# chenxuhao/GraphAIBench

Hardware: AMD Instinct MI355X
Metric: GCN-layer fwd+bwd aggregated edges/sec (higher is better)
Workload: dtype f32; 1 GPU; ogbn-products-shaped Chung-Lu graph (seed 42), GCN hidden layer 128->128 fwd+bwd (2 SpMM D=128 + 3 dense products + relu/d_relu; 2 of the products ride on the SpMMs); nv=2449029, ne_with_selfloops=125915443, D=128, parallelism=1 GPU

## Files before the change

graphaibench_amd/csrc/spmm_core.h:

```cpp
#pragma once
#include <type_traits>
#include "common.h"

namespace {

struct SpmmArgs {
  const int64_t* rowptr;
  const uint32_t* col;
  const float* rw;
  const float* ew;
  const uint32_t* rev;
  const float* in;
  float* out;
  int64_t ld;
  int64_t ldo;
  int ncols;
  int n_rows;
  int heavy_thr;
  const uint32_t* row_list;
  const uint32_t* row_order;
  int nblocks;
  int per_xcd;
  int xcd_chunk;
  uint32_t in_bytes;
  const uint32_t* col_flagged;
  int accumulate;
  int relu;
  int heads;
  int dh;
  int compact;
  int col0;
  const uint32_t* row_map;
  const float* in2;
  uint32_t n_first;
  uint32_t in2_bytes;
};

template <bool PART>
__device__ __forceinline__ int64_t out_row(const SpmmArgs& a, int64_t r) {
  if constexpr (PART) return a.row_map ? (int64_t)a.row_map[r] : r;
  else return r;
}

template <int VEC> struct VecT;
template <> struct VecT<1> { typedef float type; };
template <> struct VecT<2> { typedef float type __attribute__((ext_vector_type(2))); };
template <> struct VecT<4> { typedef float type __attribute__((ext_vector_type(4))); };
template <> struct VecT<8> { typedef float type __attribute__((ext_vector_type(8))); };

template <int VEC>
__device__ __forceinline__ typename VecT<VEC>::type vzero() {
  typename VecT<VEC>::type z;
  if constexpr (VEC == 1) z = 0.f;
  else
    for (int i = 0; i < VEC; ++i) z[i] = 0.f;
  return z;
}
template <int VEC>
__device__ __forceinline__ typename VecT<VEC>::type vrelu(typename VecT<VEC>::type v) {
  if constexpr (VEC == 1) return v > 0.f ? v : 0.f;
  else {
#pragma unroll
    for (int i = 0; i < VEC; ++i) v[i] = v[i] > 0.f ? v[i] : 0.f;
    return v;
  }
}
template <int VEC>
__device__ __forceinline__ void vacc(typename VecT<VEC>::type& acc, float w,
                                     const typename VecT<VEC>::type& x) {
  if constexpr (VEC == 1) {
    float t = w * x;
    acc = acc + t;
  } else {
#pragma unroll
    for (int i = 0; i < VEC; ++i) {
      float t = w * x[i];
      acc[i] = acc[i] + t;
    }
  }
}

__device__ __forceinline__ int logical_block(const SpmmArgs& a) {
  int b = blockIdx.x;
  if (a.per_xcd > 0) {
    const int x = b & 7, k = b >> 3;
    if (a.xcd_chunk > 0) b = ((k / a.xcd_chunk) * 8 + x) * a.xcd_chunk + (k % a.xcd_chunk);
    else b = x * a.per_xcd + k;
  }
  return b;
}

template <int WMODE>
__device__ __forceinline__ float load_edge_w(const SpmmArgs& a, int64_t e, int head = 0) {
  if constexpr (WMODE == 1) return a.ew[e];
  else if constexpr (WMODE == 2) return a.ew[a.rev[e]];
  else if constexpr (WMODE == 3) return a.ew[e * a.heads + head];
  else if constexpr (WMODE == 4) return a.ew[(int64_t)a.rev[e] * a.heads + head];
  else return 0.f;
}

typedef unsigned u2_t __attribute__((ext_vector_type(2)));
typedef unsigned u4_t __attribute__((ext_vector_type(4)));

__device__ __forceinline__ float bf16_lo(unsigned w) { return __uint_as_float(w << 16); }
__device__ __forceinline__ float bf16_hi(unsigned w) { return __uint_as_float(w & 0xffff0000u); }
template <int VEC> struct Bf16Raw;
template <> struct Bf16Raw<1> { typedef unsigned short type; };
template <> struct Bf16Raw<2> { typedef unsigned type; };
template <> struct Bf16Raw<4> { typedef u2_t type; };
template <> struct Bf16Raw<8> { typedef u4_t type; };
template <int VEC>
__device__ __forceinline__ typename VecT<VEC>::type widen_bf16(typename Bf16Raw<VEC>::type r) {
  typename VecT<VEC>::type v;
  if constexpr (VEC == 1) v = __uint_as_float((unsigned)r << 16);
  else if constexpr (VEC == 2) {
    v[0] = bf16_lo(r);
    v[1] = bf16_hi(r);
  } else {
#pragma unroll
    for (int i = 0; i < VEC / 2; ++i) {
      v[2 * i] = bf16_lo(r[i]);
      v[2 * i + 1] = bf16_hi(r[i]);
    }
  }
  return v;
}
template <int VEC, typename E>
__device__ __forceinline__ typename VecT<VEC>::type load_elems(const char* p) {
  if constexpr (sizeof(E) == 4) return *reinterpret_cast<const typename VecT<VEC>::type*>(p);
  else return widen_bf16<VEC>(*reinterpret_cast<const typename Bf16Raw<VEC>::type*>(p));
}

struct zs_t { uint32_t bits; };
constexpr int GAIB_ZS_ROW_BYTES = 384;
constexpr int GAIB_ZS_CAP = 46;
struct zs_wide_t { uint32_t bits; };
template <typename E> struct ZsTraits { static constexpr bool zs = false; static constexpr uint32_t dense_row_bytes = 0u; };
template <> struct ZsTraits<zs_t> { static constexpr bool zs = true; static constexpr uint32_t dense_row_bytes = 512u; };
template <> struct ZsTraits<zs_wide_t> { static constexpr bool zs = true; static constexpr uint32_t dense_row_bytes = 1024u; };

template <int VEC, int GM, bool PART = false, typename E = float>
struct RowGather {
  static constexpr bool BUF = GM != 0;
  static constexpr bool ZS = ZsTraits<E>::zs;
  static_assert(!PART || !ZS, "two-table gathers: fp32 or bf16 tables");
  static_assert(!ZS || (VEC == 2 && (GM == 1 || GM == 3)), "zero-suppressed tables: 8-byte lanes (128 columns), buffer addressing");
  __amdgpu_buffer_rsrc_t rsrc, rsrc2;
  const char *inb, *inb2;
  int64_t ldb;
  uint32_t n_first;
  __device__ __forceinline__ RowGather(const SpmmArgs& a) {
    inb = reinterpret_cast<const char*>(a.in);
    ldb = a.ld * (int64_t)sizeof(E);
    if constexpr (BUF) rsrc = __builtin_amdgcn_make_buffer_rsrc((void*)a.in, 0, (int)a.in_bytes, 0x00020000);
    if constexpr (PART) {
      n_first = a.in2 ? a.n_first : 0xffffffffu;
      inb2 = reinterpret_cast<const char*>(a.in2) - (int64_t)a.n_first * ldb;
      if constexpr (BUF) rsrc2 = __builtin_amdgcn_make_buffer_rsrc((void*)a.in2, 0, (int)a.in2_bytes, 0x00020000);
    }
    if constexpr (ZS) rsrc2 = __builtin_amdgcn_make_buffer_rsrc((void*)a.in2, 0, (int)a.in2_bytes, 0x00020000);
  }
  typedef typename std::conditional<ZS, u2_t, typename std::conditional<sizeof(E) == 2, typename Bf16Raw<VEC>::type,
                                                                           typename VecT<VEC>::type>::type>::type raw_t;
  static __device__ __forceinline__ typename VecT<VEC>::type widen(const raw_t& r) {
    static_assert(!ZS, "zero-suppressed tables are expanded by zs_issue / zs_select");
    if constexpr (sizeof(E) == 2) return widen_bf16<VEC>(r);
    else return r;
  }
  typedef unsigned long long zs_mask_t;
  static __device__ __forceinline__ uint32_t zs_over_bits(zs_mask_t m0, zs_mask_t m1) {
    return ((uint32_t)__builtin_popcountll(m0) + (uint32_t)(63 - GAIB_ZS_CAP)) | ((uint32_t)__builtin_popcountll(m1) + (uint32_t)(63 - GAIB_ZS_CAP));
  }
  static __device__ __forceinline__ bool zs_over(uint32_t over) { return (over & 64u) != 0; }
  static __device__ __forceinline__ void zs_issue(const raw_t& r, raw_t& p, zs_mask_t& m0, zs_mask_t& m1, uint32_t& over) {
    m0 = ((zs_mask_t)(uint32_t)__builtin_amdgcn_readlane((int)r[1], 0) << 32) | (uint32_t)__builtin_amdgcn_readlane((int)r[0], 0);
    m1 = ((zs_mask_t)(uint32_t)__builtin_amdgcn_readlane((int)r[1], 1) << 32) | (uint32_t)__builtin_amdgcn_readlane((int)r[0], 1);
    over |= zs_over_bits(m0, m1);
    const uint32_t l0 = __builtin_amdgcn_mbcnt_hi((uint32_t)(m0 >> 32), __builtin_amdgcn_mbcnt_lo((uint32_t)m0, 2u));
    const uint32_t l1 = __builtin_amdgcn_mbcnt_hi((uint32_t)(m1 >> 32), __builtin_amdgcn_mbcnt_lo((uint32_t)m1, 2u));
    p[0] = (uint32_t)__builtin_amdgcn_ds_bpermute((int)(l0 << 2), (int)r[0]);
    p[1] = (uint32_t)__builtin_amdgcn_ds_bpermute((int)(l1 << 2), (int)r[1]);
  }
  __device__ __forceinline__ typename VecT<VEC>::type zs_fix(const raw_t& p, zs_mask_t m0, zs_mask_t m1, uint32_t cvec, int idx, uint32_t voff) const {
    if (zs_over(zs_over_bits(m0, m1))) {
      const uint32_t cf = (uint32_t)__builtin_amdgcn_readlane((int)cvec, idx);
      const uint32_t cj = GM == 3 ? (cf & 0x7fffffffu) : cf;
      u2_t d;
      if (GM == 3 && (cf & 0x80000000u))
        d = __builtin_amdgcn_raw_buffer_load_b64(rsrc2, (int)voff, (int)(cj * ZsTraits<E>::dense_row_bytes), 2);
      else d = __builtin_amdgcn_raw_buffer_load_b64(rsrc2, (int)voff, (int)(cj * ZsTraits<E>::dense_row_bytes), 0);
      typename VecT<VEC>::type v;
      v[0] = __uint_as_float(d[0]);
      v[1] = __uint_as_float(d[1]);
      return v;
    }
    return zs_select(p, m0, m1);
  }
  static __device__ __forceinline__ typename VecT<VEC>::type zs_select(const raw_t& r, zs_mask_t m0, zs_mask_t m1) {
    uint32_t k0, k1;
    asm("v_cndmask_b32_e64 %0, 0, %1, %2" : "=v"(k0) : "v"(r[0]), "s"(m0));
    asm("v_cndmask_b32_e64 %0, 0, %1, %2" : "=v"(k1) : "v"(r[1]), "s"(m1));
    typename VecT<VEC>::type v;
    v[0] = __uint_as_float(k0);
    v[1] = __uint_as_float(k1);
    return v;
  }
  __device__ __forceinline__ typename VecT<VEC>::type load(uint32_t cj, uint32_t voff) const { return widen(load_raw(cj, voff)); }
  __device__ __forceinline__ raw_t load_raw(uint32_t cj, uint32_t voff) const {
    typedef typename VecT<VEC>::type vec_t;
    if constexpr (PART) {
      static_assert(GM == 0 || GM == 1, "two-table gathers: plain buffer or global loads");
      const bool second = cj >= n_first;
      if constexpr (GM == 1) {
        const int soff = (int)((second ? cj - n_first : cj) * (uint32_t)ldb);
        return load_rsrc<0>(second ? rsrc2 : rsrc, soff, voff);
      } else {
        const char* rowp = (second ? inb2 : inb) + (int64_t)cj * ldb;
        return *reinterpret_cast<const raw_t*>(rowp + voff);
      }
    } else if constexpr (ZS) {
      const int zoff = (int)(voff < (uint32_t)GAIB_ZS_ROW_BYTES ? voff : 0u);
      if constexpr (GM == 3) {
        const uint32_t c = cj & 0x7fffffffu;
        if (cj & 0x80000000u) return __builtin_amdgcn_raw_buffer_load_b64(rsrc, zoff, (int)(c * (uint32_t)GAIB_ZS_ROW_BYTES), 2);
        return __builtin_amdgcn_raw_buffer_load_b64(rsrc, zoff, (int)(c * (uint32_t)GAIB_ZS_ROW_BYTES), 0);
      } else {
        return __builtin_amdgcn_raw_buffer_load_b64(rsrc, zoff, (int)(cj * (uint32_t)GAIB_ZS_ROW_BYTES), 0);
      }
    } else if constexpr (GM == 3) {
      const uint32_t c = cj & 0x7fffffffu;
      if (cj & 0x80000000u) return load_buf<2>(c, voff);
      return load_buf<0>(c, voff);
    } else if constexpr (GM == 2) {
      return load_buf<2>(cj, voff);
    } else if constexpr (GM == 1) {
      return load_buf<0>(cj, voff);
    } else {
      const char* rowp = inb + (int64_t)cj * ldb;
      if constexpr (sizeof(E) == 2) return *reinterpret_cast<const raw_t*>(rowp + voff);
      else return *reinterpret_cast<const vec_t*>(rowp + voff);
    }
  }
  template <int AUX>
  __device__ __forceinline__ raw_t load_buf(uint32_t cj, uint32_t voff) const {
    return load_rsrc<AUX>(rsrc, (int)(cj * (uint32_t)ldb), voff);
  }
  template <int AUX>
  __device__ __forceinline__ raw_t load_rsrc(__amdgpu_buffer_rsrc_t rsrc, int soff, uint32_t voff) const {
    typedef typename VecT<VEC>::type vec_t;
    if constexpr (sizeof(E) == 2) {
      if constexpr (VEC == 1) return __builtin_amdgcn_raw_buffer_load_b16(rsrc, (int)voff, soff, AUX);
      else if constexpr (VEC == 2) return __builtin_amdgcn_raw_buffer_load_b32(rsrc, (int)voff, soff, AUX);
      else if constexpr (VEC == 4) return __builtin_amdgcn_raw_buffer_load_b64(rsrc, (int)voff, soff, AUX);
      else return __builtin_amdgcn_raw_buffer_load_b128(rsrc, (int)voff, soff, AUX);
    } else if constexpr (VEC == 1) {
      return __uint_as_float(__builtin_amdgcn_raw_buffer_load_b32(rsrc, (int)voff, soff, AUX));
    } else if constexpr (VEC == 2) {
      u2_t r = __builtin_amdgcn_raw_buffer_load_b64(rsrc, (int)voff, soff, AUX);
      vec_t v;
      v[0] = __uint_as_float(r[0]);
      v[1] = __uint_as_float(r[1]);
      return v;
    } else {
      u4_t r = __builtin_amdgcn_raw_buffer_load_b128(rsrc, (int)voff, soff, AUX);
      vec_t v;
#pragma unroll
      for (int i = 0; i < 4; ++i) v[i] = __uint_as_float(r[i]);
      return v;
    }
  }
};

#ifndef GAIB_ZS_GROUP
#define GAIB_ZS_GROUP 4
#endif

template <int G, int CT, int WMODE, int U, typename gather_t>
__device__ __forceinline__ void zs_accumulate_group(const gather_t& gather, const typename gather_t::raw_t (&x)[U][CT], int xo, uint32_t c, float w,
                                                    float roww, int j0, const uint32_t (&voff)[CT], typename VecT<2>::type (&acc)[CT]) {
  typename gather_t::zs_mask_t m0[G][CT], m1[G][CT];
  typename gather_t::raw_t p[G][CT];
  uint32_t over = 0u;
#pragma unroll
  for (int u = 0; u < G; ++u)
#pragma unroll
    for (int ct = 0; ct < CT; ++ct) gather_t::zs_issue(x[xo + u][ct], p[u][ct], m0[u][ct], m1[u][ct], over);
  if (__builtin_expect(gather_t::zs_over(over), 0)) {
#pragma unroll
    for (int u = 0; u < G; ++u) {
      const float wj = (WMODE == 0) ? roww : readlane_f(w, j0 + u);
#pragma unroll
      for (int ct = 0; ct < CT; ++ct) {
        const typename VecT<2>::type t = gather.zs_fix(p[u][ct], m0[u][ct], m1[u][ct], c, j0 + u, voff[ct]) * wj;
        acc[ct] = acc[ct] + t;
      }
    }
  } else {
#pragma unroll
    for (int u = 0; u < G; ++u) {
      const float wj = (WMODE == 0) ? roww : readlane_f(w, j0 + u);
#pragma unroll
      for (int ct = 0; ct < CT; ++ct) {
        const typename VecT<2>::type t = gather_t::zs_select(p[u][ct], m0[u][ct], m1[u][ct]) * wj;
        acc[ct] = acc[ct] + t;
      }
    }
  }
}

template <int VEC, int CT, int WMODE, int U, int BUF, bool PART = false, bool PRE = false, typename E = float>
__device__ __forceinline__ void wave_accumulate(const SpmmArgs& a, int lane, int64_t eb, int64_t ee,
                                                int64_t chunk_stride, float roww,
                                                const uint32_t (&voff)[CT],
                                                typename VecT<VEC>::type (&acc)[CT], uint32_t c_first = 0u,
                                                float w_first = 0.f) {
  static_assert((sizeof(E) == 4 && !ZsTraits<E>::zs) || WMODE < 3, "bf16 and zero-suppressed tables: single-head weights");
  typedef RowGather<VEC, BUF, PART, E> gather_t;
  const gather_t gather(a);
  typename gather_t::raw_t x[U][CT];
  constexpr bool MH = WMODE >= 3;
  int hd[CT];
  float wv[MH ? U : 1][CT];
#pragma unroll
  for (int ct = 0; ct < CT; ++ct) {
    if constexpr (MH) hd[ct] = (int)(((uint32_t)a.col0 + (voff[ct] >> 2)) / (uint32_t)a.dh);
    else hd[ct] = 0;
  }
  for (int64_t base = eb; base < ee; base += chunk_stride) {
    const int64_t rem = ee - base;
    const int n = rem < 64 ? (int)rem : 64;
    uint32_t c = 0;
    float w = 0.f;
    if (PRE && base == eb) {
      c = c_first;
      w = w_first;
    } else if (lane < n) {
      c = a.col[base + lane];
      if constexpr (WMODE == 1 || WMODE == 2) w = load_edge_w<WMODE>(a, base + lane);
    }
    int j = 0;
    for (; j + U <= n; j += U) {
#pragma unroll
      for (int u = 0; u < U; ++u) {
        const uint32_t cj = (uint32_t)__builtin_amdgcn_readlane((int)c, j + u);
#pragma unroll
        for (int ct = 0; ct < CT; ++ct) {
          x[u][ct] = gather.load_raw(cj, voff[ct]);
          if constexpr (MH) wv[u][ct] = load_edge_w<WMODE>(a, base + j + u, hd[ct]);
        }
      }
      __builtin_amdgcn_sched_barrier(0);
      if constexpr (gather_t::ZS) {
        constexpr int H = GAIB_ZS_GROUP < U ? GAIB_ZS_GROUP : U;
#pragma unroll
        for (int u = 0; u < U; u += H) zs_accumulate_group<H, CT, WMODE>(gather, x, u, c, w, roww, j + u, voff, acc);
      } else {
#pragma unroll
        for (int u = 0; u < U; ++u) {
          const float wj = (WMODE == 0) ? roww : (MH ? 0.f : readlane_f(w, j + u));
#pragma unroll
          for (int ct = 0; ct < CT; ++ct) {
            float wsel = wj;
            if constexpr (MH) wsel = wv[u][ct];
            vacc<VEC>(acc[ct], wsel, gather_t::widen(x[u][ct]));
          }
        }
      }
    }
    const int r = n - j;
    if (r > 0) {
      int jj = j;
#pragma unroll
      for (int p = U / 2; p >= 1; p >>= 1) {
        if (r & p) {
#pragma unroll
          for (int u = 0; u < p; ++u) {
            const uint32_t cj = (uint32_t)__builtin_amdgcn_readlane((int)c, jj + u);
#pragma unroll
            for (int ct = 0; ct < CT; ++ct) x[p + u][ct] = gather.load_raw(cj, voff[ct]);
          }
          jj += p;
        }
      }
      __builtin_amdgcn_sched_barrier(0);
      jj = j;
#pragma unroll
      for (int p = U / 2; p >= 1; p >>= 1) {
        if (r & p) {
          if constexpr (gather_t::ZS) {
            if (p >= GAIB_ZS_GROUP) {
#pragma unroll
              for (int u = 0; u < p; u += GAIB_ZS_GROUP)
                zs_accumulate_group<GAIB_ZS_GROUP, CT, WMODE>(gather, x, p + u, c, w, roww, jj + u, voff, acc);
            } else if (p == 8) zs_accumulate_group<8, CT, WMODE>(gather, x, p, c, w, roww, jj, voff, acc);
            else if (p == 4) zs_accumulate_group<4, CT, WMODE>(gather, x, p, c, w, roww, jj, voff, acc);
            else if (p == 2) zs_accumulate_group<2, CT, WMODE>(gather, x, p, c, w, roww, jj, voff, acc);
            else zs_accumulate_group<1, CT, WMODE>(gather, x, p, c, w, roww, jj, voff, acc);
          } else {
#pragma unroll
            for (int u = 0; u < p; ++u) {
              const float wj = (WMODE == 0) ? roww : (MH ? 0.f : readlane_f(w, jj + u));
#pragma unroll
              for (int ct = 0; ct < CT; ++ct) {
                float wh = wj;
                if constexpr (MH) wh = load_edge_w<WMODE>(a, base + jj + u, hd[ct]);
                vacc<VEC>(acc[ct], wh, gather_t::widen(x[p + u][ct]));
              }
            }
          }
          jj += p;
        }
      }
    }
  }
}

}
```

graphaibench_amd/csrc/spmm_kernels.h:

```cpp
#pragma once
#include <algorithm>
#include "spmm_core.h"

namespace {

template <int VEC, int CT, int WMODE, int U, int BUF, bool PART = false, typename E = float>
__global__ __launch_bounds__(256) void spmm_w64_kernel(SpmmArgs a) {
  typedef typename VecT<VEC>::type vec_t;
  const int lane = threadIdx.x & 63;
  const int lb = logical_block(a);
  if (lb >= a.nblocks) return;
  int row = lb * 4 + (threadIdx.x >> 6);
  if (row >= a.n_rows) return;
  row = __builtin_amdgcn_readfirstlane(row);
  const int64_t e0 = a.rowptr[row], e1 = a.rowptr[row + 1];
  if (e1 - e0 > (int64_t)a.heavy_thr) return;
  bool colok[CT];
  uint32_t voff[CT];
  vec_t acc[CT];
#pragma unroll
  for (int ct = 0; ct < CT; ++ct) {
    colok[ct] = (lane + ct * 64) * VEC < a.ncols;
    voff[ct] = colok[ct] ? (uint32_t)((lane + ct * 64) * VEC * (int)sizeof(E)) : 0u;
    acc[ct] = vzero<VEC>();
  }
  const float roww = (WMODE == 0) ? a.rw[row] : 0.f;
  float* o = a.out + out_row<PART>(a, row) * a.ldo + lane * VEC;
  if (a.accumulate) {
#pragma unroll
    for (int ct = 0; ct < CT; ++ct)
      if (colok[ct]) acc[ct] = *reinterpret_cast<const vec_t*>(o + ct * 64 * VEC);
  }
  wave_accumulate<VEC, CT, WMODE, U, BUF, PART, false, E>(a, lane, e0, e1, 64, roww, voff, acc);
#pragma unroll
  for (int ct = 0; ct < CT; ++ct)
    if (colok[ct]) *reinterpret_cast<vec_t*>(o + ct * 64 * VEC) = a.relu ? vrelu<VEC>(acc[ct]) : acc[ct];
}

constexpr int HEAVY_WAVES = 16;
template <int VEC, int CT, int WMODE, int U, int BUF, bool PART = false, typename E = float>
__global__ __launch_bounds__(HEAVY_WAVES * 64) void spmm_heavy_kernel(SpmmArgs a) {
  typedef typename VecT<VEC>::type vec_t;
  extern __shared__ __attribute__((aligned(16))) float red[];
  const int lane = threadIdx.x & 63;
  const int wave = threadIdx.x >> 6;
  const int slot = (int)a.row_order[blockIdx.x];
  const int row = (int)a.row_list[slot];
  const int64_t e0 = a.rowptr[row], e1 = a.rowptr[row + 1];
  uint32_t voff[CT];
  vec_t acc[CT];
#pragma unroll
  for (int ct = 0; ct < CT; ++ct) {
    const bool ok = (lane + ct * 64) * VEC < a.ncols;
    voff[ct] = ok ? (uint32_t)((lane + ct * 64) * VEC * (int)sizeof(E)) : 0u;
    acc[ct] = vzero<VEC>();
  }
  const float roww = (WMODE == 0) ? a.rw[row] : 0.f;
  wave_accumulate<VEC, CT, WMODE, U, BUF, PART, false, E>(a, lane, e0 + (int64_t)wave * 64, e1,
                                                          (int64_t)HEAVY_WAVES * 64, roww, voff, acc);
  constexpr int W = CT * 64 * VEC;
#pragma unroll
  for (int ct = 0; ct < CT; ++ct)
    *reinterpret_cast<vec_t*>(&red[wave * W + (ct * 64 + lane) * VEC]) = acc[ct];
  __syncthreads();
  float* orow = a.out + (a.compact ? (int64_t)slot : out_row<PART>(a, row)) * a.ldo;
  for (int c = threadIdx.x; c < a.ncols; c += HEAVY_WAVES * 64) {
    float s = a.accumulate ? orow[c] + red[c] : red[c];
#pragma unroll
    for (int w = 1; w < HEAVY_WAVES; ++w) s = s + red[w * W + c];
    orow[c] = (a.relu && !(s > 0.f)) ? 0.f : s;
  }
}

template <int VEC, int G, int WMODE, typename E = float>
__global__ __launch_bounds__(256) void spmm_sub_kernel(SpmmArgs a) {
  typedef typename VecT<VEC>::type vec_t;
  constexpr int RPW = 64 / G;
  constexpr int U = 4;
  const int lane = threadIdx.x & 63;
  const int sub = lane / G, sl = lane % G;
  const int lb = logical_block(a);
  if (lb >= a.nblocks) return;
  const int64_t row = ((int64_t)lb * 4 + (threadIdx.x >> 6)) * RPW + sub;
  int64_t e0 = 0, e1 = 0;
  bool active = row < a.n_rows;
  if (active) {
    e0 = a.rowptr[row];
    e1 = a.rowptr[row + 1];
    if (e1 - e0 > (int64_t)a.heavy_thr) { active = false; e1 = e0; }
  }
  const bool colok = sl * VEC < a.ncols;
  vec_t acc = vzero<VEC>();
  if (a.accumulate && active && colok) acc = *reinterpret_cast<const vec_t*>(a.out + row * a.ldo + sl * VEC);
  const float roww = (WMODE == 0 && active) ? a.rw[row] : 0.f;
  const int head = (WMODE >= 3 && colok) ? (sl * VEC) / a.dh : 0;
  const float* inl = a.in + sl * VEC;
  const char* inl_e = reinterpret_cast<const char*>(a.in) + sl * VEC * (int)sizeof(E);
  for (int64_t e = e0; e < e1; e += U) {
    uint32_t cj[U];
    float wj[U];
    vec_t x[U];
#pragma unroll
    for (int u = 0; u < U; ++u) {
      const bool ok = e + u < e1;
      cj[u] = ok ? a.col[e + u] : 0u;
      wj[u] = (WMODE == 0) ? roww : (ok ? load_edge_w<WMODE>(a, e + u, head) : 0.f);
    }
#pragma unroll
    for (int u = 0; u < U; ++u) {
      const bool ok = e + u < e1;
      if constexpr (sizeof(E) == 2)
        x[u] = (ok && colok) ? load_elems<VEC, E>(inl_e + (int64_t)cj[u] * a.ld * 2) : vzero<VEC>();
      else
        x[u] = (ok && colok) ? *reinterpret_cast<const vec_t*>(inl + (int64_t)cj[u] * a.ld) : vzero<VEC>();
    }
#pragma unroll
    for (int u = 0; u < U; ++u)
      if (e + u < e1) vacc<VEC>(acc, wj[u], x[u]);
  }
  if (active && colok) *reinterpret_cast<vec_t*>(a.out + row * a.ldo + sl * VEC) = a.relu ? vrelu<VEC>(acc) : acc;
}

template <int VEC, int CT, int WMODE, int U, int BUF, bool PART = false, typename E = float>
int launch_w64_u(gaib_ctx* ctx, const gaib_graph* g, SpmmArgs a) {
  constexpr double EB = sizeof(E);
  if (g->n_heavy > 0) {
    SpmmArgs h = a;
    h.row_list = g->heavy_rows;
    h.row_order = g->heavy_rows + g->n_heavy;
    size_t lds = sizeof(float) * HEAVY_WAVES * CT * 64 * VEC;
    ProfScope ps(ctx, sizeof(E) == 2 ? "spmm_bf16_heavy" : "spmm_heavy",
                 gaib_alg_spmm_bytes((double)g->heavy_edges, (double)g->n_heavy, a.ncols, WMODE == 0 ? 0 : 4, a.accumulate ? 2 : 1, EB),
                 2.0 * g->heavy_edges * a.ncols, a.ncols);
    constexpr int UH = (WMODE >= 3 && U * CT * VEC > 16) ? (U / 2 > 4 ? U / 2 : 4) : U;
    spmm_heavy_kernel<VEC, CT, WMODE, UH, BUF, PART, E><<<dim3((unsigned)g->n_heavy), HEAVY_WAVES * 64, lds,
                                                         ctx->stream>>>(h);
    GAIB_LAUNCH_CHECK();
  }
  a.nblocks = (int)cdiv64(a.n_rows, 4);
  unsigned grid = (unsigned)a.nblocks;
  if (ctx->spmm_xcd_swizzle && a.nblocks >= 64) {
    a.per_xcd = (int)cdiv64(a.nblocks, 8);
    if (ctx->spmm_xcd_swizzle == 2 && a.nblocks >= 8 * 64) {
      a.xcd_chunk = 64;
      a.per_xcd = (int)(cdiv64(a.per_xcd, 64) * 64);
    }
    grid = (unsigned)a.per_xcd * 8u;
  }
  if (grid > 0) {
    const double e_l = (double)g->ne - (g->n_heavy > 0 ? (double)g->heavy_edges : 0.0), r_l = (double)a.n_rows - (double)g->n_heavy;
    ProfScope ps(ctx, sizeof(E) == 2 ? (!PART ? "spmm_bf16_light" : (a.in2 ? "part_bf16_light_2t" : (a.accumulate ? "part_bf16_light_acc" : "part_bf16_light")))
                                     : (!PART ? "spmm_light" : (a.in2 ? "part_light_2t" : (a.accumulate ? "part_light_acc" : "part_light"))),
                 gaib_alg_spmm_bytes(e_l, r_l, a.ncols, WMODE == 0 ? 0 : 4, a.accumulate ? 2 : 1, EB), 2.0 * e_l * a.ncols, a.ncols);
    spmm_w64_kernel<VEC, CT, WMODE, U, BUF, PART, E><<<dim3(grid), 256, 0, ctx->stream>>>(a);
    GAIB_LAUNCH_CHECK();
  }
  return GAIB_OK;
}

template <int VEC, int CT, int WMODE, typename E = float>
int launch_w64(gaib_ctx* ctx, const gaib_graph* g, SpmmArgs a) {
  constexpr int U = (VEC * CT >= 8) ? 4 : (VEC * CT >= 4 ? 8 : 16);
  int gm = (a.in_bytes != 0 && ctx->spmm_addr_mode != 2) ? 1 : 0;
  if (gm == 1 && ctx->spmm_gather_mode == 2) gm = 2;
  if (gm == 1 && ctx->spmm_gather_mode == 3 && a.col_flagged) {
    gm = 3;
    a.col = a.col_flagged;
  }
  if constexpr (U > 8) {
    if (ctx->spmm_unroll == 8) {
      switch (gm) {
        case 0: return launch_w64_u<VEC, CT, WMODE, 8, 0, false, E>(ctx, g, a);
        case 2: return launch_w64_u<VEC, CT, WMODE, 8, 2, false, E>(ctx, g, a);
        case 3: return launch_w64_u<VEC, CT, WMODE, 8, 3, false, E>(ctx, g, a);
        default: return launch_w64_u<VEC, CT, WMODE, 8, 1, false, E>(ctx, g, a);
      }
    }
  }
  switch (gm) {
    case 0: return launch_w64_u<VEC, CT, WMODE, U, 0, false, E>(ctx, g, a);
    case 2: return launch_w64_u<VEC, CT, WMODE, U, 2, false, E>(ctx, g, a);
    case 3: return launch_w64_u<VEC, CT, WMODE, U, 3, false, E>(ctx, g, a);
    default: return launch_w64_u<VEC, CT, WMODE, U, 1, false, E>(ctx, g, a);
  }
}

template <int VEC, int G, int WMODE, typename E = float>
int launch_sub(gaib_ctx* ctx, const gaib_graph* g, SpmmArgs a) {
  if (g->n_heavy > 0) {
    SpmmArgs h = a;
    h.row_list = g->heavy_rows;
    h.row_order = g->heavy_rows + g->n_heavy;
    size_t lds = sizeof(float) * HEAVY_WAVES * 64 * VEC;
    ProfScope ps(ctx, sizeof(E) == 2 ? "spmm_bf16_heavy" : "spmm_heavy",
                 gaib_alg_spmm_bytes((double)g->heavy_edges, (double)g->n_heavy, a.ncols, WMODE == 0 ? 0 : 4, a.accumulate ? 2 : 1,
                                     (double)sizeof(E)), 2.0 * g->heavy_edges * a.ncols, a.ncols);
    constexpr int UH = VEC >= 8 ? 4 : 8;
    spmm_heavy_kernel<VEC, 1, WMODE, UH, 0, false, E><<<dim3((unsigned)g->n_heavy), HEAVY_WAVES * 64, lds,
                                                         ctx->stream>>>(h);
    GAIB_LAUNCH_CHECK();
  }
  constexpr int RPW = 64 / G;
  a.nblocks = (int)cdiv64(a.n_rows, 4 * RPW);
  unsigned grid = (unsigned)a.nblocks;
  if (ctx->spmm_xcd_swizzle && a.nblocks >= 64) {
    a.per_xcd = (int)cdiv64(a.nblocks, 8);
    grid = (unsigned)a.per_xcd * 8u;
  }
  if (grid > 0) {
    const double e_l = (double)g->ne - (g->n_heavy > 0 ? (double)g->heavy_edges : 0.0), r_l = (double)a.n_rows - (double)g->n_heavy;
    ProfScope ps(ctx, sizeof(E) == 2 ? "spmm_bf16_sub" : "spmm_sub",
                 gaib_alg_spmm_bytes(e_l, r_l, a.ncols, WMODE == 0 ? 0 : 4, a.accumulate ? 2 : 1, (double)sizeof(E)), 2.0 * e_l * a.ncols,
                 a.ncols);
    spmm_sub_kernel<VEC, G, WMODE, E><<<dim3(grid), 256, 0, ctx->stream>>>(a);
    GAIB_LAUNCH_CHECK();
  }
  return GAIB_OK;
}

template <int VEC, int WMODE>
int dispatch_ct(gaib_ctx* ctx, const gaib_graph* g, const SpmmArgs& a, int lanes) {
  if (lanes <= 64) return launch_w64<VEC, 1, WMODE>(ctx, g, a);
  if (lanes <= 128) return launch_w64<VEC, 2, WMODE>(ctx, g, a);
  if constexpr (VEC == 4) {
    gaib_set_error("spmm: %d 16-byte lanes in one launch (internal: the slab width is 128 lanes at VEC = 4)", lanes);
    return GAIB_ERR_INVALID;
  } else {
    return launch_w64<VEC, 4, WMODE>(ctx, g, a);
  }
}

template <int VEC, int WMODE>
int dispatch_sub(gaib_ctx* ctx, const gaib_graph* g, const SpmmArgs& a, int lanes) {
  if (lanes <= 1) return launch_sub<VEC, 1, WMODE>(ctx, g, a);
  if (lanes <= 2) return launch_sub<VEC, 2, WMODE>(ctx, g, a);
  if (lanes <= 4) return launch_sub<VEC, 4, WMODE>(ctx, g, a);
  if (lanes <= 8) return launch_sub<VEC, 8, WMODE>(ctx, g, a);
  if (lanes <= 16) return launch_sub<VEC, 16, WMODE>(ctx, g, a);
  return launch_sub<VEC, 32, WMODE>(ctx, g, a);
}

template <int WMODE>
int dispatch_vec(gaib_ctx* ctx, const gaib_graph* g, const SpmmArgs& a0, int len) {
  const uintptr_t al = (uintptr_t)a0.in | (uintptr_t)a0.out;
  int vmax = 1;
  if (len % 4 == 0 && (al & 15) == 0) vmax = 4;
  else if (len % 2 == 0 && (al & 7) == 0) vmax = 2;
  if (WMODE >= 3) {
    while (vmax > 1 && a0.dh % vmax != 0) vmax >>= 1;
  }
  int variant = ctx->spmm_variant;
  const int lanes_max = (len + vmax - 1) / vmax;
  bool use_sub = false;
  int vec = vmax;
  if (len <= 64) vec = 1;
  else if (len <= 256 && vmax >= 2) vec = 2;
  else if (len <= 128) vec = 1;
  if (WMODE >= 3 && a0.dh % vec != 0) vec = 1;
  if (variant == 1) { use_sub = false; vec = 1; }
  if (variant == 2 && vmax >= 2) { use_sub = false; vec = 2; }
  if (variant == 4 && vmax >= 4) { use_sub = false; vec = 4; }
  if (variant == 32 && lanes_max <= 32) { use_sub = true; vec = vmax; }
  if (use_sub) {
    SpmmArgs a = a0;
    a.ncols = len;
    const int lanes = (len + vec - 1) / vec;
    if (vec == 4) return dispatch_sub<4, WMODE>(ctx, g, a, lanes);
    if (vec == 2) return dispatch_sub<2, WMODE>(ctx, g, a, lanes);
    return dispatch_sub<1, WMODE>(ctx, g, a, lanes);
  }
  const int slab = (vec == 4 ? 128 : 256) * vec;
  for (int c0 = 0; c0 < len; c0 += slab) {
    SpmmArgs a = a0;
    a.in = a0.in + c0;
    a.out = a0.out + c0;
    a.col0 = c0;
    if (a.in_bytes) a.in_bytes -= (uint32_t)(c0 * 4);
    a.ncols = (len - c0 < slab) ? (len - c0) : slab;
    const int lanes = (a.ncols + vec - 1) / vec;
    int rc;
    if (vec == 4) rc = dispatch_ct<4, WMODE>(ctx, g, a, lanes);
    else if (vec == 2) rc = dispatch_ct<2, WMODE>(ctx, g, a, lanes);
    else rc = dispatch_ct<1, WMODE>(ctx, g, a, lanes);
    if (rc != GAIB_OK) return rc;
  }
  return GAIB_OK;
}

struct FuseArgs {
  const float* wt;
  float* y;
  int64_t ldy;
  int n_out;
  int relu;
  const float* heavy_agg;
  const uint32_t* heavy_rows;
  int n_heavy;
  int* tile_counter;
  const float* agg_in;
  const float* wt2;
  const float* rows2;
  int ldw;
  int y_accum;
  int overlaps_transfer;
  int tile_xcd;
};

static int tile_xcd_arg(gaib_ctx* ctx, gaib_graph* g) {
  int v = ctx->spmm_tile_xcd;
  if (v < 0) {
    if (gaib_graph_ensure_locality(ctx, g) != GAIB_OK) return 0;
    v = g->near_frac >= 0.25f ? 1024 : 0;
  }
  if (v <= 0) return 0;
  if (v == 1) v = 16;
  int sh = 0;
  while ((2 << sh) <= v) ++sh;
  return sh + 1;
}

typedef float f32x4_t __attribute__((ext_vector_type(4)));
constexpr int FUSE_ROWS = 16;
constexpr int FUSE_WAVES = 16;

template <int VEC, int WMODE, int U, int GM, int STRIP, bool DUAL, bool FLAT = false, bool YACC = false, bool PART = false,
          bool RING = false, bool AFFINE = false, bool PREF = false, typename E = float>
__global__ __launch_bounds__(FUSE_WAVES * 64) void spmm_gemm_kernel(SpmmArgs a, FuseArgs f) {
  typedef typename VecT<VEC>::type vec_t;
  typedef RowGather<VEC, GM, PART, E> gather_t;
  constexpr int K = 64 * VEC;
  constexpr int KQ = K / 4;
  constexpr int LDT = K + 4;
  constexpr int HALF = STRIP;
  constexpr int NPASS = FUSE_ROWS / STRIP;
  extern __shared__ __attribute__((aligned(16))) float fuse_lds[];
  const int lane = threadIdx.x & 63;
  const int wave = threadIdx.x >> 6;
  const int n_pad = (f.n_out + 15) & ~15;
  float* wl = fuse_lds;
  float* wl2 = fuse_lds + n_pad * LDT;
  float* tile = fuse_lds + (DUAL ? 2 : 1) * n_pad * LDT + wave * (HALF * LDT);
  for (int t = threadIdx.x; t < n_pad * K; t += FUSE_WAVES * 64) {
    const int n = t / K, k = t % K;
    const bool in = n < f.n_out && k < a.ncols;
    wl[n * LDT + k] = in ? f.wt[(int64_t)n * f.ldw + k] : 0.f;
    if constexpr (DUAL) wl2[n * LDT + k] = in ? f.wt2[(int64_t)n * f.ldw + k] : 0.f;
  }
  __syncthreads();
  const int i = lane & 15, kq = lane >> 4;
  const bool colok = lane * VEC < a.ncols;
  auto store_row = [&](vec_t* p, const vec_t& v) { __builtin_nontemporal_store(v, p); };
  const uint32_t voff[1] = {colok ? (uint32_t)(lane * VEC * (int)sizeof(E)) : 0u};
  const int ntiles = (a.n_rows + FUSE_ROWS - 1) / FUSE_ROWS;
  const int tsh = AFFINE ? f.tile_xcd - 1 : 0;
  int own = AFFINE ? (int)(blockIdx.x & 7) : 0;
  int k_next = 0, k_left = 0;
  const int nwaves4 = ((int)gridDim.x * FUSE_WAVES * 4) / 8 > 0 ? ((int)gridDim.x * FUSE_WAVES * 4) / 8 : 1;
  const int per_xcd_tiles = (ntiles + 7) / 8;
  const int n_chunks = AFFINE ? (ntiles + (1 << tsh) - 1) >> tsh : 0;
  for (;;) {
    if (k_left == 0) {
      int want = 1;
// ... 553 lines not shown
```

Before: 14.69 billion edges/s.

## Software-pipeline zero-suppressed gathers by refilling buffers during group accumulation

In the zero-suppressed gather path with U=16, the edge loop now preloads the first 16 neighbor rows. After each 4-wide group's decode is issued, it starts loading the matching rows of the next chunk, so memory latency overlaps with accumulation. The remainder (tail) loads are also placed into freed slots during the last full chunk. The heavy-row kernel opts out and keeps the old loop. This costs more register pressure and a more complex tail-slot mapping, which could lower occupancy.

```diff
diff --git a/graphaibench_amd/csrc/spmm_core.h b/graphaibench_amd/csrc/spmm_core.h
--- a/graphaibench_amd/csrc/spmm_core.h
+++ b/graphaibench_amd/csrc/spmm_core.h
@@ -275,9 +275,13 @@
 #define GAIB_ZS_GROUP 4
 #endif
 
-template <int G, int CT, int WMODE, int U, typename gather_t>
+struct ZsNoRefill {
+  __device__ __forceinline__ void operator()() const {}
+};
+template <int G, int CT, int WMODE, int U, typename gather_t, typename refill_t = ZsNoRefill>
 __device__ __forceinline__ void zs_accumulate_group(const gather_t& gather, const typename gather_t::raw_t (&x)[U][CT], int xo, uint32_t c, float w,
-                                                    float roww, int j0, const uint32_t (&voff)[CT], typename VecT<2>::type (&acc)[CT]) {
+                                                    float roww, int j0, const uint32_t (&voff)[CT], typename VecT<2>::type (&acc)[CT],
+                                                    const refill_t& refill = refill_t()) {
   typename gather_t::zs_mask_t m0[G][CT], m1[G][CT];
   typename gather_t::raw_t p[G][CT];
   uint32_t over = 0u;
@@ -285,6 +289,10 @@
   for (int u = 0; u < G; ++u)
 #pragma unroll
     for (int ct = 0; ct < CT; ++ct) gather_t::zs_issue(x[xo + u][ct], p[u][ct], m0[u][ct], m1[u][ct], over);
+  if constexpr (!std::is_same<refill_t, ZsNoRefill>::value) {
+    refill();
+    __builtin_amdgcn_sched_barrier(0);
+  }
   if (__builtin_expect(gather_t::zs_over(over), 0)) {
 #pragma unroll
     for (int u = 0; u < G; ++u) {
@@ -308,7 +316,7 @@
   }
 }
 
-template <int VEC, int CT, int WMODE, int U, int BUF, bool PART = false, bool PRE = false, typename E = float>
+template <int VEC, int CT, int WMODE, int U, int BUF, bool PART = false, bool PRE = false, typename E = float, bool ROLL = true>
 __device__ __forceinline__ void wave_accumulate(const SpmmArgs& a, int lane, int64_t eb, int64_t ee,
                                                 int64_t chunk_stride, float roww,
                                                 const uint32_t (&voff)[CT],
@@ -339,7 +347,56 @@
       if constexpr (WMODE == 1 || WMODE == 2) w = load_edge_w<WMODE>(a, base + lane);
     }
     int j = 0;
-    for (; j + U <= n; j += U) {
+    bool tail_requested = false;
+    constexpr bool ROLLING = ROLL && gather_t::ZS && GAIB_ZS_GROUP == 4 && U == 4 * GAIB_ZS_GROUP;
+    if constexpr (ROLLING) {
+      constexpr int H = GAIB_ZS_GROUP;
+      if (n >= U) {
+#pragma unroll
+        for (int u = 0; u < U; ++u) {
+          const uint32_t cj = (uint32_t)__builtin_amdgcn_readlane((int)c, u);
+#pragma unroll
+          for (int ct = 0; ct < CT; ++ct) x[u][ct] = gather.load_raw(cj, voff[ct]);
+        }
+        __builtin_amdgcn_sched_barrier(0);
+        for (; j + 2 * U <= n; j += U) {
+#pragma unroll
+          for (int u = 0; u < U; u += H)
+            zs_accumulate_group<H, CT, WMODE>(gather, x, u, c, w, roww, j + u, voff, acc, [&]() {
+#pragma unroll
+              for (int v = 0; v < H; ++v) {
+                const uint32_t cj = (uint32_t)__builtin_amdgcn_readlane((int)c, j + U + u + v);
+#pragma unroll
+                for (int ct = 0; ct < CT; ++ct) x[u + v][ct] = gather.load_raw(cj, voff[ct]);
+              }
+            });
+        }
+        const int r = n - j - U;
+        const int j8 = j + U, j4 = j8 + (r & 8), j2 = j4 + (r & 4), j1 = j2 + (r & 2);
+        auto request = [&](int xo, int cnt, int e) {
+#pragma unroll
+          for (int v = 0; v < cnt; ++v) {
+            const uint32_t cj = (uint32_t)__builtin_amdgcn_readlane((int)c, e + v);
+#pragma unroll
+            for (int ct = 0; ct < CT; ++ct) x[xo + v][ct] = gather.load_raw(cj, voff[ct]);
+          }
+        };
+        static_assert(U == 4 * H && H == 4, "the tail's pieces are placed for four groups of four");
+#pragma unroll
+        for (int u = 0; u < U; u += H)
+          zs_accumulate_group<H, CT, WMODE>(gather, x, u, c, w, roww, j + u, voff, acc, [&]() {
+            if (u == 0) {
+              if (r & 2) request(2, 2, j2);
+              if (r & 1) request(1, 1, j1);
+            } else if (u == H) {
+              if (r & 4) request(4, 4, j4);
+            } else if (r & 8) request(u, H, j8 + (u - 2 * H));
+          });
+        j += U;
+        tail_requested = true;
+      }
+    }
+    for (; j + U <= n && !ROLLING; j += U) {
 #pragma unroll
       for (int u = 0; u < U; ++u) {
         const uint32_t cj = (uint32_t)__builtin_amdgcn_readlane((int)c, j + u);
@@ -370,16 +427,18 @@
     const int r = n - j;
     if (r > 0) {
       int jj = j;
-#pragma unroll
-      for (int p = U / 2; p >= 1; p >>= 1) {
-        if (r & p) {
-#pragma unroll
-          for (int u = 0; u < p; ++u) {
-            const uint32_t cj = (uint32_t)__builtin_amdgcn_readlane((int)c, jj + u);
-#pragma unroll
-            for (int ct = 0; ct < CT; ++ct) x[p + u][ct] = gather.load_raw(cj, voff[ct]);
+      if (!tail_requested) {
+#pragma unroll
+        for (int p = U / 2; p >= 1; p >>= 1) {
+          if (r & p) {
+#pragma unroll
+            for (int u = 0; u < p; ++u) {
+              const uint32_t cj = (uint32_t)__builtin_amdgcn_readlane((int)c, jj + u);
+#pragma unroll
+              for (int ct = 0; ct < CT; ++ct) x[p + u][ct] = gather.load_raw(cj, voff[ct]);
+            }
+            jj += p;
           }
-          jj += p;
         }
       }
       __builtin_amdgcn_sched_barrier(0);
diff --git a/graphaibench_amd/csrc/spmm_kernels.h b/graphaibench_amd/csrc/spmm_kernels.h
--- a/graphaibench_amd/csrc/spmm_kernels.h
+++ b/graphaibench_amd/csrc/spmm_kernels.h
@@ -56,8 +56,8 @@
     acc[ct] = vzero<VEC>();
   }
   const float roww = (WMODE == 0) ? a.rw[row] : 0.f;
-  wave_accumulate<VEC, CT, WMODE, U, BUF, PART, false, E>(a, lane, e0 + (int64_t)wave * 64, e1,
-                                                          (int64_t)HEAVY_WAVES * 64, roww, voff, acc);
+  wave_accumulate<VEC, CT, WMODE, U, BUF, PART, false, E, false>(a, lane, e0 + (int64_t)wave * 64, e1,
+                                                                 (int64_t)HEAVY_WAVES * 64, roww, voff, acc);
   constexpr int W = CT * 64 * VEC;
 #pragma unroll
   for (int ct = 0; ct < CT; ++ct)
```

New measurement: 14.84 billion edges/s (median of 5 runs). +1.0%, better.
